# facebookresearch/metamorph

Measured on AMD Instinct MI355X. Metric: train tokens/sec (LLaMA-3-8B + SigLIP-SO400M, seq2048, 256 img toks), whole job, higher is better.
Workload: dtype bf16

## Files before the change

### metamorph_amd/build.py

```python
from __future__ import annotations

import hashlib
import os
import subprocess
import sys

PKG = os.path.dirname(os.path.abspath(__file__))
CSRC = os.path.join(PKG, "csrc")
LIBDIR = os.path.join(PKG, "lib")
LIB = os.path.join(LIBDIR, "libmm355.so")
SOURCES = ["gemm_bf16.hip", "rowwise.hip", "elementwise.hip", "attn.hip", "attn2.hip", "attn4.hip", "attn4_bwd.hip", "decode.hip", "attn_decode.hip", "decode_w8.hip", "decode_w4.hip", "decode_kv8.hip", "attn_extend.hip", "attn_extend_shared.hip", "gemm_w8.hip", "gemm_w4.hip", "greedy.hip", "sample.hip", "logits.hip", "beam.hip", "losses.hip", "linear_ce.hip"]
HEADERS = ["mm355_common.h", "gemm_common.h", "splitk.h", "gemm_wq.h", "decode_wq.h", "attn2.h", "attn_tile.h", "rowsum.h", "argrows.h"] + sorted(
    os.path.join(d, f) for d in ("attn4_gen", "attn4_bwd_gen")
    for f in os.listdir(os.path.join(CSRC, d)) if f.endswith(".inc"))
BASE_FLAGS = ["--offload-arch=gfx950", "-O3", "-std=c++17", "-fPIC", "-Wno-unused-result"]
FLAGS = BASE_FLAGS + ["-mllvm", "-amdgpu-mfma-vgpr-form=1"]
FLAGS_OF = {f: BASE_FLAGS + ["-mllvm", "-amdgpu-spill-vgpr-to-agpr=0"] for f in ("attn4.hip", "attn4_bwd.hip")}


def _hipcc():
    for c in (os.environ.get("HIPCC"), "/opt/rocm/bin/hipcc", "hipcc"):
        if c and (os.path.isabs(c) and os.path.exists(c) or not os.path.isabs(c)):
            return c
    raise RuntimeError("hipcc not found")


def _digest():
    h = hashlib.sha256()
    for f in SOURCES + HEADERS:
        h.update(open(os.path.join(CSRC, f), "rb").read())
    h.update(open(os.path.join(os.path.dirname(PKG), "include", "mm355.h"), "rb").read())
    h.update(" ".join(FLAGS).encode())
    h.update(repr(sorted(FLAGS_OF.items())).encode())
    return h.hexdigest()


def build(force: bool = False, verbose: bool = True) -> str:
    os.makedirs(LIBDIR, exist_ok=True)
    stamp = os.path.join(LIBDIR, "libmm355.stamp")
    dig = _digest()
    if not force and os.path.exists(LIB) and os.path.exists(stamp) and open(stamp).read().strip() == dig:
        return LIB
    hipcc = _hipcc()
    objs = []
    procs = []
    for src in SOURCES:
        obj = os.path.join(LIBDIR, src.replace(".hip", ".o"))
        cmd = [hipcc, *FLAGS_OF.get(src, FLAGS), "-c", os.path.join(CSRC, src), "-o", obj]
        if verbose:
            print("[mm355 build]", " ".join(cmd), flush=True)
        procs.append((src, subprocess.Popen(cmd, stdout=subprocess.PIPE, stderr=subprocess.STDOUT)))
        objs.append(obj)
    for src, p in procs:
        out, _ = p.communicate()
        if p.returncode != 0:
            raise RuntimeError(f"hipcc failed on {src}:\n{out.decode(errors='replace')}")
    cmd = [hipcc, "--offload-arch=gfx950", "-shared", "-fPIC", "-o", LIB, *objs]
    if verbose:
        print("[mm355 build]", " ".join(cmd), flush=True)
    subprocess.check_call(cmd)
    with open(stamp, "w") as f:
        f.write(dig)
    return LIB


if __name__ == "__main__":
    print(build(force="--force" in sys.argv))
```

### metamorph_amd/csrc/gemm_bf16.hip

```cpp
#include "gemm_common.h"
#include "splitk.h"
#include <type_traits>
#include <cstdlib>

namespace {

MM_DEV void gemm_epilogue_swiglu(f32x4 (&acc)[8][4], const GemmArgs& a, unsigned char* smem, int m0, int tn, int wm, int wn, int wave, int lane) {
    constexpr int TN = 64;
    const int fr = lane & 15, fq = lane >> 4;
    const int M = a.M, I = (int)a.res_mod;
    float* stg = (float*)smem + wave * (16 * TN);
    const int row_l = lane >> 2, k4 = lane & 3;
    uint16_t* gu = (uint16_t*)a.C;
    uint16_t* act = (uint16_t*)a.res;
    const int ch0 = tn * 128 + wn * 32;
#pragma unroll
    for (int i = 0; i < 8; ++i) {
        __builtin_amdgcn_fence(__ATOMIC_RELEASE, "wavefront");
        __builtin_amdgcn_wave_barrier();
#pragma unroll
        for (int j = 0; j < 4; ++j)
#pragma unroll
            for (int r = 0; r < 4; ++r) stg[(fq * 4 + r) * TN + j * 16 + fr] = acc[i][j][r];
        __builtin_amdgcn_fence(__ATOMIC_RELEASE, "wavefront");
        __builtin_amdgcn_wave_barrier();
        const int grow = m0 + wm * 128 + i * 16 + row_l;
        if (grow < M) {
            float g[8], u[8], o[8];
            const f32x4 g0 = *(const f32x4*)(stg + row_l * TN + k4 * 8), g1 = *(const f32x4*)(stg + row_l * TN + k4 * 8 + 4);
            const f32x4 u0 = *(const f32x4*)(stg + row_l * TN + 32 + k4 * 8), u1 = *(const f32x4*)(stg + row_l * TN + 32 + k4 * 8 + 4);
            g[0] = g0.x; g[1] = g0.y; g[2] = g0.z; g[3] = g0.w; g[4] = g1.x; g[5] = g1.y; g[6] = g1.z; g[7] = g1.w;
            u[0] = u0.x; u[1] = u0.y; u[2] = u0.z; u[3] = u0.w; u[4] = u1.x; u[5] = u1.y; u[6] = u1.z; u[7] = u1.w;
            const u32x4 gp = pack8(g), up = pack8(u);
            const int ch = ch0 + k4 * 8;
            *(u32x4*)(gu + (int64_t)grow * a.ldc + ch) = gp;
            *(u32x4*)(gu + (int64_t)grow * a.ldc + I + ch) = up;
            float gb[8], ub[8];
            unpack8(gp, gb);
            unpack8(up, ub);
#pragma unroll
            for (int e = 0; e < 8; ++e) o[e] = round_bf(gb[e] / (1.0f + __expf(-gb[e]))) * ub[e];
            *(u32x4*)(act + (int64_t)grow * a.ldr + ch) = pack8(o);
        }
    }
}

constexpr int SWB_TROW = 144;
constexpr int SWB_T = 3 * 32 * SWB_TROW;
constexpr int SWB_LDS = 32768 + 8 * SWB_T;
MM_DEV void gemm_epilogue_swiglu_bwd(f32x4 (&acc)[8][4], const GemmArgs& a, unsigned char* smem, int m0, int n0, int wm, int wn, int wave, int lane) {
    constexpr int TN = 64, PF = 4;
    typedef __attribute__((ext_vector_type(4))) short s16x4;
    typedef __attribute__((address_space(3))) s16x4* lds4_t;
    const int fr = lane & 15, fq = lane >> 4;
    const int M = a.M, I = a.N;
    float* stg = (float*)smem + wave * (16 * TN);
    unsigned char* tile = smem + 32768 + wave * SWB_T;
    const int row_l = lane >> 2, k4 = lane & 3;
    const uint16_t* gu = a.res;
    uint16_t* dgu = (uint16_t*)a.C;
    const int c_wave = n0 + wn * 64;
    if (c_wave >= I) return;
    const int row0 = m0 + wm * 128 + row_l;
    u32x4 gq[PF][2], uq[PF][2];
    auto fetch = [&](int i, int slot) {
        const int grow = row0 + i * 16;
#pragma unroll
        for (int j8 = 0; j8 < 2; ++j8) {
            const int64_t ro = (int64_t)min(grow, M - 1) * a.ldr + c_wave + k4 * 16 + j8 * 8;
            gq[slot][j8] = *(const u32x4*)(gu + ro);
            uq[slot][j8] = *(const u32x4*)(gu + ro + I);
        }
    };
#pragma unroll
    for (int i = 0; i < PF; ++i) fetch(i, i);
#pragma unroll
    for (int ib = 0; ib < 4; ++ib) {
#pragma unroll
        for (int half = 0; half < 2; ++half) {
            const int i = ib * 2 + half;
            __builtin_amdgcn_fence(__ATOMIC_RELEASE, "wavefront");
            __builtin_amdgcn_wave_barrier();
#pragma unroll
            for (int j = 0; j < 4; ++j)
// ... 580 lines not shown
template <int ABL = 0>
__global__ __launch_bounds__(512) void gemm_pp_kernel(GemmArgs a) {
    extern __shared__ __attribute__((aligned(16))) unsigned char smem[];
#ifdef MM355_PP_PERSIST
    const int total = a.ntm * a.ntn;
    for (int bid = blockIdx.x; bid < total; bid += gridDim.x) {
        gemm_pp_tile<ABL>(a, bid, smem);
        __syncthreads();
    }
#else
    gemm_pp_tile<ABL>(a, blockIdx.x, smem);
#endif
}

__global__ __launch_bounds__(512) void gemm_pp_pair_kernel(GemmArgs a0, GemmArgs a1, int n0) {
    extern __shared__ __attribute__((aligned(16))) unsigned char smem[];
    const int bid = blockIdx.x;
    if (bid < n0) gemm_pp_tile(a0, bid, smem);
    else gemm_pp_tile(a1, bid - n0, smem);
}

template <int BM, int BN, int WM, int WN, bool GLDS, int PIPE>
int launch_gemm(GemmArgs a, hipStream_t s);

constexpr int PP_LDS = 2 * (256 + 256) * 128;

int64_t pp_prepare(GemmArgs& a) {
    a.ntm = (a.M + 255) / 256;
    a.ntn = (a.N + 255) / 256;
    a.gm = 4;
    return (int64_t)a.ntm * a.ntn;
}

template <int ABL = 0>
int launch_gemm_pp_t(GemmArgs a, hipStream_t s) {
    static std::atomic<uint64_t> lds_ok{0};
    if (mm_ensure_dynamic_lds((const void*)gemm_pp_kernel<ABL>, PP_LDS, lds_ok) != MM355_OK) return MM355_ELAUNCH;
    const int64_t total = pp_prepare(a);
    if (total <= 0 || total > 0x7fffffff) return MM355_EINVAL;
#ifdef MM355_PP_PERSIST
    hipLaunchKernelGGL((gemm_pp_kernel<ABL>), dim3((unsigned)std::min<int64_t>(total, MM355_PP_PERSIST)), dim3(512), PP_LDS, s, a);
#else
    hipLaunchKernelGGL((gemm_pp_kernel<ABL>), dim3((unsigned)total), dim3(512), PP_LDS, s, a);
#endif
    return mm_launch_status();
}

int launch_gemm_pp_pair(GemmArgs a0, GemmArgs a1, hipStream_t s) {
    static std::atomic<uint64_t> lds_ok{0};
    if (mm_ensure_dynamic_lds((const void*)gemm_pp_pair_kernel, PP_LDS, lds_ok) != MM355_OK) return MM355_ELAUNCH;
    const int64_t n0 = pp_prepare(a0), n1 = pp_prepare(a1);
    if (n0 <= 0 || n1 <= 0 || n0 + n1 > 0x7fffffff) return MM355_EINVAL;
    hipLaunchKernelGGL(gemm_pp_pair_kernel, dim3((unsigned)(n0 + n1)), dim3(512), PP_LDS, s, a0, a1, (int)n0);
    return mm_launch_status();
}

bool pp_eligible(const GemmArgs& a) {
    if (a.K < 128 || (a.K & 127)) return false;
    const int64_t ea = (256 * a.lda + a.K) * 2;
    const int64_t eb = (256 * a.ldb + a.K) * 2;
    return ea < 0x7fffffffLL && eb < 0x7fffffffLL;
}

int launch_gemm_pp(GemmArgs a, hipStream_t s) {
    if (!pp_eligible(a)) return launch_gemm<256, 256, 2, 4, true, 1>(a, s);
    return launch_gemm_pp_t(a, s);
}

template <int BM, int BN, int WM, int WN, bool GLDS, int PIPE = 0>
int launch_gemm(GemmArgs a, hipStream_t s) {
    constexpr int STAGE = (BM + BN) * 128;
    constexpr int LDS = 2 * STAGE;
    auto kern = gemm_nt_kernel<BM, BN, WM, WN, GLDS, PIPE>;
    static std::atomic<uint64_t> lds_ok{0};
    if (mm_ensure_dynamic_lds((const void*)kern, LDS, lds_ok) != MM355_OK) return MM355_ELAUNCH;
    a.ntm = (a.M + BM - 1) / BM;
    a.ntn = (a.N + BN - 1) / BN;
    const int64_t total = (int64_t)a.ntm * a.ntn;
    if (total <= 0 || total > 0x7fffffff) return MM355_EINVAL;
    hipLaunchKernelGGL(kern, dim3((unsigned)total), dim3(WM * WN * 64), LDS, s, a);
    return mm_launch_status();
}

__global__ __launch_bounds__(256) void transpose_kernel(const uint16_t* __restrict__ in, int64_t ld_in, int rows, int cols,
                                                        uint16_t* __restrict__ out, int64_t ld_out) {
    __shared__ uint16_t tile[64][64 + 2];
    const int r0 = blockIdx.y * 64, c0 = blockIdx.x * 64;
    const int tid = threadIdx.x;
#pragma unroll
    for (int i = 0; i < 2; ++i) {
        const int v = tid + i * 256, r = v >> 3, c = (v & 7) * 8;
        const int gr = r0 + r, gc = c0 + c;
        uint16_t tmp[8];
        if (gr < rows && gc + 8 <= cols) {
            *(u32x4*)tmp = *(const u32x4*)(in + (int64_t)gr * ld_in + gc);
        } else {
#pragma unroll
            for (int e = 0; e < 8; ++e) tmp[e] = (gr < rows && gc + e < cols) ? in[(int64_t)gr * ld_in + gc + e] : (uint16_t)0;
        }
#pragma unroll
        for (int e = 0; e < 8; ++e) tile[r][c + e] = tmp[e];
    }
    __syncthreads();
#pragma unroll
    for (int i = 0; i < 2; ++i) {
        const int v = tid + i * 256, c = v >> 3, r = (v & 7) * 8;
        const int gc = c0 + c, gr = r0 + r;
        if (gc >= cols) continue;
        uint16_t tmp[8];
#pragma unroll
        for (int e = 0; e < 8; ++e) tmp[e] = tile[r + e][c];
        if (gr + 8 <= rows && ((ld_out & 7) == 0)) {
            *(u32x4*)(out + (int64_t)gc * ld_out + gr) = *(const u32x4*)tmp;
        } else {
            for (int e = 0; e < 8; ++e)
                if (gr + e < rows) out[(int64_t)gc * ld_out + gr + e] = tmp[e];
        }
    }
}

__global__ __launch_bounds__(256) void colsum_kernel(const uint16_t* __restrict__ x, int64_t ld, int M, int N, float* __restrict__ out) {
    __shared__ float part[4][64];
    const int cq = threadIdx.x & 63, rp = threadIdx.x >> 6;
    const int c = blockIdx.x * 64 + cq;
    float s = 0.f;
    if (c < N)
        for (int r = rp; r < M; r += 4) s += bf2f(x[(int64_t)r * ld + c]);
    part[rp][cq] = s;
    __syncthreads();
    if (rp == 0 && c < N) out[c] += (part[0][cq] + part[1][cq]) + (part[2][cq] + part[3][cq]);
}

__global__ __launch_bounds__(1024) void colsum8_kernel(const uint16_t* __restrict__ x, int64_t ld, int M, int N, float* __restrict__ out) {
    __shared__ float part[128][65];
    const int cg = threadIdx.x & 7, rp = threadIdx.x >> 3;
    const int c0 = blockIdx.x * 64 + cg * 8;
    float s[8] = {0.f, 0.f, 0.f, 0.f, 0.f, 0.f, 0.f, 0.f};
    if (c0 < N)
        for (int r = rp; r < M; r += 128) {
            float f[8];
            unpack8(*(const u32x4*)(x + (int64_t)r * ld + c0), f);
#pragma unroll
            for (int e = 0; e < 8; ++e) s[e] += f[e];
        }
#pragma unroll
    for (int e = 0; e < 8; ++e) part[rp][cg * 8 + e] = s[e];
    __syncthreads();
    const int c = blockIdx.x * 64 + threadIdx.x;
    if (threadIdx.x < 64 && c < N) {
        float t = 0.f;
        for (int p = 0; p < 128; ++p) t += part[p][threadIdx.x];
        out[c] += t;
    }
}

}

namespace {
__global__ __launch_bounds__(256) void splitk_reduce_kernel(const float* __restrict__ part, int S, int M, int N, const uint16_t* __restrict__ res,
                                                            int64_t ldr, uint16_t* __restrict__ out, int64_t ldc) {
    const int nv = N >> 3;
    const int64_t total = (int64_t)M * nv, plane = (int64_t)M * N;
    for (int64_t i = blockIdx.x * 256ll + threadIdx.x; i < total; i += (int64_t)gridDim.x * 256) {
        const int m = (int)(i / nv), c = (int)(i % nv) * 8;
        float v[8];
        const float* p = part + (int64_t)m * N + c;
        const f32x4 a0 = *(const f32x4*)p, a1 = *(const f32x4*)(p + 4);
        v[0] = a0.x; v[1] = a0.y; v[2] = a0.z; v[3] = a0.w; v[4] = a1.x; v[5] = a1.y; v[6] = a1.z; v[7] = a1.w;
        for (int s = 1; s < S; ++s) {
            const f32x4 b0 = *(const f32x4*)(p + s * plane), b1 = *(const f32x4*)(p + s * plane + 4);
            v[0] += b0.x; v[1] += b0.y; v[2] += b0.z; v[3] += b0.w; v[4] += b1.x; v[5] += b1.y; v[6] += b1.z; v[7] += b1.w;
        }
        if (res) {
            float r[8];
            unpack8(*(const u32x4*)(res + (int64_t)m * ldr + c), r);
#pragma unroll
            for (int e = 0; e < 8; ++e) v[e] += r[e];
        }
        *(u32x4*)(out + (int64_t)m * ldc + c) = pack8(v);
    }
}

MM_DEV void splitk_sum8(const float* __restrict__ p, int S, int64_t plane, float (&v)[8]) {
    const f32x4 a0 = *(const f32x4*)p, a1 = *(const f32x4*)(p + 4);
    v[0] = a0.x; v[1] = a0.y; v[2] = a0.z; v[3] = a0.w; v[4] = a1.x; v[5] = a1.y; v[6] = a1.z; v[7] = a1.w;
    int s = 1;
    for (; s + 3 < S; s += 4) {
        f32x4 b0[4], b1[4];
#pragma unroll
        for (int j = 0; j < 4; ++j) { b0[j] = *(const f32x4*)(p + (s + j) * plane); b1[j] = *(const f32x4*)(p + (s + j) * plane + 4); }
#pragma unroll
        for (int j = 0; j < 4; ++j) {
            v[0] += b0[j].x; v[1] += b0[j].y; v[2] += b0[j].z; v[3] += b0[j].w; v[4] += b1[j].x; v[5] += b1[j].y; v[6] += b1[j].z; v[7] += b1[j].w;
        }
    }
    for (; s < S; ++s) {
        const f32x4 b0 = *(const f32x4*)(p + s * plane), b1 = *(const f32x4*)(p + s * plane + 4);
        v[0] += b0.x; v[1] += b0.y; v[2] += b0.z; v[3] += b0.w; v[4] += b1.x; v[5] += b1.y; v[6] += b1.z; v[7] += b1.w;
    }
}
template <int VPT>
// ... 277 lines not shown
        return rc != MM355_OK ? rc : mm355_rope_kv_append(qkv, ld_qkv, M, Hq, Hkv, d, cos_t, sin_t, positions, k_cache, v_cache, ld_kv, batch_stride_kv, stream);
    }
    int slices = 0;
    const int rc = splitk_partials(X, ldx, Wqkv, ldw, M, N, K, S, workspace, workspace_floats, (hipStream_t)stream, slices);
    if (rc != MM355_OK) return rc;
    return mm_splitk_reduce_rope_append(workspace, slices, M, Hq, Hkv, d, qkv, ld_qkv, cos_t, sin_t, positions, k_cache, v_cache, ld_kv,
                                        batch_stride_kv, (hipStream_t)stream);
}

extern "C" int mm355_gemm_num_variants(void) { return 14; }

extern "C" int mm355_gemm_bf16(const mm355_bf16* A, int64_t lda, const mm355_bf16* B, int64_t ldb, void* C, int64_t ldc,
                               int64_t M, int64_t N, int64_t K, const mm355_bf16* bias, const mm355_bf16* residual,
                               int64_t ldr, int64_t res_row_mod, uint32_t flags, int variant, void* stream) {
    (void)hipGetLastError();
    if (!A || !B || !C || M <= 0 || N <= 0 || K <= 0) return MM355_EINVAL;
    if ((K & 7) || (lda & 7) || (ldb & 7) || !mm_aligned16(A) || !mm_aligned16(B) || !mm_aligned16(C)) return MM355_EINVAL;
    if (M > 0x7fffffff || N > 0x7fffffff || K > 0x7fffffff) return MM355_EINVAL;
    if ((flags & MM355_GEMM_BIAS) && (!bias || !mm_aligned16(bias))) return MM355_EINVAL;
    if ((flags & MM355_GEMM_RESIDUAL) && (!residual || !mm_aligned16(residual))) return MM355_EINVAL;
    if ((flags & MM355_GEMM_GELU_ERF) && (flags & MM355_GEMM_GELU_TANH)) return MM355_EINVAL;
    GemmArgs a = {};
    a.A = A; a.B = B; a.C = C; a.bias = bias; a.res = residual;
    a.lda = lda; a.ldb = ldb; a.ldc = ldc; a.ldr = ldr; a.res_mod = res_row_mod;
    a.M = (int)M; a.N = (int)N; a.K = (int)K; a.flags = flags; a.ntm = a.ntn = 0;
    hipStream_t s = (hipStream_t)stream;
    const bool dma_ok = (K % 64) == 0;
    if (variant == 0) {
        const int64_t t256 = ((M + 255) / 256) * ((N + 255) / 256);
        const int64_t t128 = ((M + 127) / 128) * ((N + 127) / 128);
        if (dma_ok) {
            variant = (t256 >= 200) ? 11 : 2;
            if (variant == 2 && t128 < 224 && M > 64 && t128 * 2 >= 64) variant = 9;
        } else variant = 1;
    }
    if (!dma_ok && variant != 1) return MM355_EUNSUPPORTED;
    switch (variant) {
        case 1: return launch_gemm<128, 128, 2, 2, false>(a, s);
        case 2: return launch_gemm<128, 128, 2, 2, true>(a, s);
        case 7: return launch_gemm<256, 256, 2, 4, true, 1>(a, s);
        case 9: return launch_gemm<64, 128, 1, 4, true>(a, s);
        case 11: return launch_gemm_pp(a, s);
#ifdef MM355_ABLATIONS
        case 91: return launch_gemm_pp_t<1>(a, s);
        case 92: return launch_gemm_pp_t<2>(a, s);
        case 93: return launch_gemm_pp_t<3>(a, s);
#endif
        default: return MM355_EUNSUPPORTED;
    }
}

namespace {
int pair_problem(GemmArgs& a, const mm355_bf16* A, int64_t lda, const mm355_bf16* B, int64_t ldb, void* C, int64_t ldc,
                 int64_t M, int64_t N, int64_t K, uint32_t flags) {
    if (!A || !B || !C || M <= 0 || N <= 0 || K <= 0) return MM355_EINVAL;
    if ((K & 7) || (lda & 7) || (ldb & 7) || !mm_aligned16(A) || !mm_aligned16(B) || !mm_aligned16(C)) return MM355_EINVAL;
    if (M > 0x7fffffff || N > 0x7fffffff || K > 0x7fffffff) return MM355_EINVAL;
    if (flags & ~(MM355_GEMM_ACCUMULATE | MM355_GEMM_OUT_F32)) return MM355_EINVAL;
    a.A = A; a.B = B; a.C = C; a.bias = nullptr; a.res = nullptr;
    a.lda = lda; a.ldb = ldb; a.ldc = ldc; a.ldr = 0; a.res_mod = 0;
    a.M = (int)M; a.N = (int)N; a.K = (int)K; a.flags = flags; a.ntm = a.ntn = 0;
    return pp_eligible(a) ? MM355_OK : MM355_EUNSUPPORTED;
}
}

extern "C" int mm355_gemm_pair_bf16(const mm355_bf16* A0, int64_t lda0, const mm355_bf16* B0, int64_t ldb0, void* C0, int64_t ldc0,
                                    int64_t M0, int64_t N0, int64_t K0, uint32_t flags0,
                                    const mm355_bf16* A1, int64_t lda1, const mm355_bf16* B1, int64_t ldb1, void* C1, int64_t ldc1,
                                    int64_t M1, int64_t N1, int64_t K1, uint32_t flags1, void* stream) {
    (void)hipGetLastError();
    GemmArgs a0, a1;
    int rc = pair_problem(a0, A0, lda0, B0, ldb0, C0, ldc0, M0, N0, K0, flags0);
    if (rc != MM355_OK) return rc;
    rc = pair_problem(a1, A1, lda1, B1, ldb1, C1, ldc1, M1, N1, K1, flags1);
    if (rc != MM355_OK) return rc;
    return launch_gemm_pp_pair(a0, a1, (hipStream_t)stream);
}

extern "C" int mm355_transpose_bf16(const mm355_bf16* in, int64_t ld_in, int64_t rows, int64_t cols, mm355_bf16* out,
                                    int64_t ld_out, void* stream) {
    (void)hipGetLastError();
    if (!in || !out || rows <= 0 || cols <= 0 || (ld_in & 7) || !mm_aligned16(in) || !mm_aligned16(out)) return MM355_EINVAL;
    if (ld_out < rows || rows > 0x7fffffff || cols > 0x7fffffff) return MM355_EINVAL;
    dim3 grid((unsigned)((cols + 63) / 64), (unsigned)((rows + 63) / 64));
    hipLaunchKernelGGL(transpose_kernel, grid, dim3(256), 0, (hipStream_t)stream, in, ld_in, (int)rows, (int)cols, out, ld_out);
    return mm_launch_status();
}

extern "C" int mm355_gemm_swiglu_bf16(const mm355_bf16* X, int64_t ldx, const mm355_bf16* Wgu, int64_t ldw, mm355_bf16* gu, int64_t ld_gu,
                                      mm355_bf16* act, int64_t ld_act, int64_t M, int64_t I, int64_t K, void* stream) {
    (void)hipGetLastError();
    if (!X || !Wgu || !gu || !act || M <= 0 || I <= 0 || K <= 0) return MM355_EINVAL;
    if ((ldx & 7) || (ldw & 7) || (ld_gu & 7) || (ld_act & 7) || !mm_aligned16(X) || !mm_aligned16(Wgu) || !mm_aligned16(gu) || !mm_aligned16(act))
        return MM355_EINVAL;
    if (M > 0x7fffffff || I > 0x3fffffff || K > 0x7fffffff) return MM355_EINVAL;
    if ((I & 127) || K < 128 || (K & 127) || (2 * I * ldw + K) * 2 >= 0x7fffffffLL || (256 * ldx + K) * 2 >= 0x7fffffffLL) return MM355_EUNSUPPORTED;
    GemmArgs a = {};
    a.A = X; a.B = Wgu; a.C = gu; a.bias = nullptr; a.res = act;
    a.lda = ldx; a.ldb = ldw; a.ldc = ld_gu; a.ldr = ld_act; a.res_mod = I;
    a.M = (int)M; a.N = (int)(2 * I); a.K = (int)K; a.flags = 0; a.ntm = a.ntn = 0;
    static std::atomic<uint64_t> lds_ok{0};
    if (mm_ensure_dynamic_lds((const void*)gemm_pp_swiglu_kernel, PP_LDS, lds_ok) != MM355_OK) return MM355_ELAUNCH;
    const int64_t total = pp_prepare(a);
    if (total <= 0 || total > 0x7fffffff) return MM355_EINVAL;
    hipLaunchKernelGGL(gemm_pp_swiglu_kernel, dim3((unsigned)total), dim3(512), PP_LDS, (hipStream_t)stream, a);
    return mm_launch_status();
}

extern "C" int mm355_gemm_rope_bf16(const mm355_bf16* X, int64_t ldx, const mm355_bf16* Wqkv, int64_t ldw, mm355_bf16* qkv, int64_t ld_qkv,
                                    const mm355_bf16* cos_t, const mm355_bf16* sin_t, const int32_t* pos_offset,
                                    int64_t M, int64_t N, int64_t K, int64_t L, int64_t n_rot, void* stream) {
    (void)hipGetLastError();
    if (!X || !Wqkv || !qkv || !cos_t || !sin_t || M <= 0 || N <= 0 || K <= 0 || L <= 0 || n_rot < 0 || n_rot > N) return MM355_EINVAL;
    if ((ldx & 7) || (ldw & 7) || (ld_qkv & 7) || !mm_aligned16(X) || !mm_aligned16(Wqkv) || !mm_aligned16(qkv) || !mm_aligned16(cos_t) || !mm_aligned16(sin_t))
        return MM355_EINVAL;
    if (M > 0x7fffffff || N > 0x7fffffff || K > 0x7fffffff || L > 0x7fffffff) return MM355_EINVAL;
    if ((N & 255) || (n_rot & 127) || K < 128 || (K & 127) || (256 * ldx + K) * 2 >= 0x7fffffffLL || (256 * ldw + K) * 2 >= 0x7fffffffLL) return MM355_EUNSUPPORTED;
    GemmArgs a = {};
    a.A = X; a.B = Wqkv; a.C = qkv; a.bias = (const uint16_t*)pos_offset; a.res = nullptr;
    a.lda = ldx; a.ldb = ldw; a.ldc = ld_qkv; a.ldr = 0; a.res_mod = n_rot;
    a.M = (int)M; a.N = (int)N; a.K = (int)K; a.flags = 0; a.ntm = a.ntn = 0;
    a.aux0 = (uint16_t*)cos_t; a.aux1 = (uint16_t*)sin_t; a.ld_aux = L;
    static std::atomic<uint64_t> lds_ok{0};
    if (mm_ensure_dynamic_lds((const void*)gemm_pp_rope_kernel, PP_LDS, lds_ok) != MM355_OK) return MM355_ELAUNCH;
    const int64_t total = pp_prepare(a);
    if (total <= 0 || total > 0x7fffffff) return MM355_EINVAL;
    hipLaunchKernelGGL(gemm_pp_rope_kernel, dim3((unsigned)total), dim3(512), PP_LDS, (hipStream_t)stream, a);
    return mm_launch_status();
}

extern "C" int mm355_gemm_swiglu_bwd_bf16(const mm355_bf16* dY, int64_t ldy, const mm355_bf16* WdT, int64_t ldw, const mm355_bf16* gu, int64_t ld_gu,
                                          mm355_bf16* dgu, int64_t ld_dgu, mm355_bf16* actT, mm355_bf16* dguT, int64_t ldT,
                                          int64_t M, int64_t I, int64_t K, void* stream) {
    (void)hipGetLastError();
    if (!dY || !WdT || !gu || !dgu || !actT || !dguT || M <= 0 || I <= 0 || K <= 0) return MM355_EINVAL;
    if ((ldy & 7) || (ldw & 7) || (ld_gu & 7) || (ld_dgu & 7) || (ldT & 7) || ldT < M || !mm_aligned16(dY) || !mm_aligned16(WdT) || !mm_aligned16(gu)
        || !mm_aligned16(dgu) || !mm_aligned16(actT) || !mm_aligned16(dguT))
        return MM355_EINVAL;
    if (M > 0x7fffffff || I > 0x3fffffff || K > 0x7fffffff) return MM355_EINVAL;
    if ((I & 63) || (M & 7) || K < 128 || (K & 127) || (256 * ldy + K) * 2 >= 0x7fffffffLL || (256 * ldw + K) * 2 >= 0x7fffffffLL) return MM355_EUNSUPPORTED;
    GemmArgs a = {};
    a.A = dY; a.B = WdT; a.C = dgu; a.bias = nullptr; a.res = gu;
    a.lda = ldy; a.ldb = ldw; a.ldc = ld_dgu; a.ldr = ld_gu; a.res_mod = 0;
    a.M = (int)M; a.N = (int)I; a.K = (int)K; a.flags = 0; a.ntm = a.ntn = 0;
    a.aux0 = actT; a.aux1 = dguT; a.ld_aux = ldT;
    static std::atomic<uint64_t> lds_ok{0};
    if (mm_ensure_dynamic_lds((const void*)gemm_pp_swiglu_bwd_kernel, SWB_LDS, lds_ok) != MM355_OK) return MM355_ELAUNCH;
    const int64_t total = pp_prepare(a);
    if (total <= 0 || total > 0x7fffffff) return MM355_EINVAL;
    hipLaunchKernelGGL(gemm_pp_swiglu_bwd_kernel, dim3((unsigned)total), dim3(512), SWB_LDS, (hipStream_t)stream, a);
    return mm_launch_status();
}

extern "C" int mm355_colsum_bf16(const mm355_bf16* dY, int64_t ld, int64_t M, int64_t N, float* db_f32, void* stream) {
    (void)hipGetLastError();
    if (!dY || !db_f32 || M <= 0 || N <= 0) return MM355_EINVAL;
    if (M > 0x7fffffff || N > 0x7fffffff) return MM355_EINVAL;
    if (!(N & 7) && !(ld & 7) && mm_aligned16(dY) && M >= 256)
        hipLaunchKernelGGL(colsum8_kernel, dim3((unsigned)((N + 63) / 64)), dim3(1024), 0, (hipStream_t)stream, dY, ld, (int)M, (int)N, db_f32);
    else
        hipLaunchKernelGGL(colsum_kernel, dim3((unsigned)((N + 63) / 64)), dim3(256), 0, (hipStream_t)stream, dY, ld, (int)M, (int)N, db_f32);
    return mm_launch_status();
}
```

### metamorph_amd/csrc/rowwise.hip

```cpp
#include "mm355_common.h"
#include "rowsum.h"
#include <type_traits>

namespace {

constexpr int NT = 256;

template <int VPT>
__global__ __launch_bounds__(NT) void rmsnorm_fwd_kernel(const uint16_t* __restrict__ x, const uint16_t* __restrict__ w,
                                                         uint16_t* __restrict__ y, float* __restrict__ rstd_out, int h, float eps) {
    __shared__ float red[NT / 64];
    const int64_t row = blockIdx.x;
    const int nv = h >> 3;
    const uint16_t* xr = x + row * h;
    float xv[VPT][8];
    float ss = 0.f;
#pragma unroll
    for (int i = 0; i < VPT; ++i) {
        const int v = threadIdx.x + i * NT;
        if (v < nv) {
            unpack8(*(const u32x4*)(xr + v * 8), xv[i]);
#pragma unroll
            for (int e = 0; e < 8; ++e) ss += xv[i][e] * xv[i][e];
        }
    }
    ss = block_sum<NT>(ss, red);
    const float rstd = rsqrtf(ss / (float)h + eps);
    if (rstd_out && threadIdx.x == 0) rstd_out[row] = rstd;
#pragma unroll
    for (int i = 0; i < VPT; ++i) {
        const int v = threadIdx.x + i * NT;
        if (v < nv) {
            float wv[8], o[8];
            unpack8(*(const u32x4*)(w + v * 8), wv);
#pragma unroll
            for (int e = 0; e < 8; ++e) o[e] = wv[e] * round_bf(xv[i][e] * rstd);
            *(u32x4*)(y + row * h + v * 8) = pack8(o);
        }
    }
}

__global__ __launch_bounds__(256) void rmsnorm_apply_t_kernel(const uint16_t* __restrict__ x, const uint16_t* __restrict__ w,
                                                              const float* __restrict__ rstd, int M, int h,
                                                              uint16_t* __restrict__ out, int64_t ld_out) {
    __shared__ uint16_t tile[64][64 + 2];
    const int r0 = blockIdx.y * 64, c0 = blockIdx.x * 64;
    const int tid = threadIdx.x;
#pragma unroll
    for (int i = 0; i < 2; ++i) {
        const int v = tid + i * 256, r = v >> 3, c = (v & 7) * 8;
        const int gr = r0 + r, gc = c0 + c;
        uint16_t tmp[8];
        if (gr < M && gc + 8 <= h) {
            float xv[8], wv[8], o[8];
            unpack8(*(const u32x4*)(x + (int64_t)gr * h + gc), xv);
            unpack8(*(const u32x4*)(w + gc), wv);
            const float rs = rstd[gr];
#pragma unroll
            for (int e = 0; e < 8; ++e) o[e] = wv[e] * round_bf(xv[e] * rs);
            *(u32x4*)tmp = pack8(o);
        } else {
#pragma unroll
            for (int e = 0; e < 8; ++e) tmp[e] = 0;
        }
#pragma unroll
        for (int e = 0; e < 8; ++e) tile[r][c + e] = tmp[e];
    }
    __syncthreads();
#pragma unroll
    for (int i = 0; i < 2; ++i) {
        const int v = tid + i * 256, c = v >> 3, r = (v & 7) * 8;
        const int gc = c0 + c, gr = r0 + r;
        if (gc >= h) continue;
        uint16_t tmp[8];
#pragma unroll
        for (int e = 0; e < 8; ++e) tmp[e] = tile[r + e][c];
        if (gr + 8 <= M && ((ld_out & 7) == 0)) {
            *(u32x4*)(out + (int64_t)gc * ld_out + gr) = *(const u32x4*)tmp;
        } else {
            for (int e = 0; e < 8; ++e)
                if (gr + e < M) out[(int64_t)gc * ld_out + gr + e] = tmp[e];
        }
    }
}

template <int VPT>
__global__ __launch_bounds__(NT) void rmsnorm_bwd_kernel(const uint16_t* __restrict__ dy, const uint16_t* __restrict__ x,
                                                         const uint16_t* __restrict__ w, const uint16_t* __restrict__ dres,
                                                         uint16_t* __restrict__ dx, float* __restrict__ dw,
                                                         float* __restrict__ ws, int M, int h, float eps, int rows_per_block) {
    __shared__ float red[NT / 64];
    const int nv = h >> 3;
    float wv[VPT][8], dwacc[VPT][8];
#pragma unroll
    for (int i = 0; i < VPT; ++i) {
        const int v = threadIdx.x + i * NT;
#pragma unroll
        for (int e = 0; e < 8; ++e) { dwacc[i][e] = 0.f; wv[i][e] = 0.f; }
        if (v < nv) unpack8(*(const u32x4*)(w + v * 8), wv[i]);
    }
    const int r0 = blockIdx.x * rows_per_block, r1 = min(M, r0 + rows_per_block);
    for (int row = r0; row < r1; ++row) {
        const uint16_t* xr = x + (int64_t)row * h;
        const uint16_t* gr = dy + (int64_t)row * h;
        float xv[VPT][8], gv[VPT][8];
        float ss = 0.f;
#pragma unroll
        for (int i = 0; i < VPT; ++i) {
            const int v = threadIdx.x + i * NT;
            if (v < nv) {
                unpack8(*(const u32x4*)(xr + v * 8), xv[i]);
                unpack8(*(const u32x4*)(gr + v * 8), gv[i]);
#pragma unroll
                for (int e = 0; e < 8; ++e) ss += xv[i][e] * xv[i][e];
            }
        }
        ss = block_sum<NT>(ss, red);
        const float rstd = rsqrtf(ss / (float)h + eps);
        float dot = 0.f;
#pragma unroll
        for (int i = 0; i < VPT; ++i) {
            const int v = threadIdx.x + i * NT;
            if (v < nv) {
#pragma unroll
                for (int e = 0; e < 8; ++e) {
                    const float xh = xv[i][e] * rstd;
                    dwacc[i][e] += gv[i][e] * round_bf(xh);
                    gv[i][e] *= wv[i][e];
                    dot += gv[i][e] * xh;
                }
            }
        }
        dot = block_sum<NT>(dot, red) / (float)h;
#pragma unroll
        for (int i = 0; i < VPT; ++i) {
            const int v = threadIdx.x + i * NT;
            if (v < nv) {
                float o[8];
                if (dres) unpack8(*(const u32x4*)(dres + (int64_t)row * h + v * 8), o);
                else {
#pragma unroll
                    for (int e = 0; e < 8; ++e) o[e] = 0.f;
                }
#pragma unroll
                for (int e = 0; e < 8; ++e) o[e] += rstd * (gv[i][e] - xv[i][e] * rstd * dot);
                *(u32x4*)(dx + (int64_t)row * h + v * 8) = pack8(o);
            }
        }
    }
    if (ws) {
        float* wr = ws + (int64_t)blockIdx.x * h;
#pragma unroll
        for (int i = 0; i < VPT; ++i) {
            const int v = threadIdx.x + i * NT;
            if (v < nv) {
                *(f32x4*)(wr + v * 8) = f32x4{dwacc[i][0], dwacc[i][1], dwacc[i][2], dwacc[i][3]};
                *(f32x4*)(wr + v * 8 + 4) = f32x4{dwacc[i][4], dwacc[i][5], dwacc[i][6], dwacc[i][7]};
            }
        }
    } else if (dw) {
#pragma unroll
        for (int i = 0; i < VPT; ++i) {
            const int v = threadIdx.x + i * NT;
            if (v < nv) {
#pragma unroll
                for (int e = 0; e < 8; ++e) atomicAdd(dw + v * 8 + e, dwacc[i][e]);
// ... 314 lines not shown
    else { lerp_src(oy, si, so, y0, y1, ly); lerp_src(ox, si, so, x0, x1, lx); }
    const int64_t base = (int64_t)n * si * si * C;
    const int64_t o00 = base + (int64_t)(y0 * si + x0) * C, o01 = base + (int64_t)(y0 * si + x1) * C;
    const int64_t o10 = base + (int64_t)(y1 * si + x0) * C, o11 = base + (int64_t)(y1 * si + x1) * C;
    const uint16_t* g = dy + (int64_t)tok * C;
    auto interp = [&](int v, float* r) {
        float a[8], bq[8], c[8], d[8];
        unpack8(*(const u32x4*)(in + o00 + v * 8), a);
        unpack8(*(const u32x4*)(in + o01 + v * 8), bq);
        unpack8(*(const u32x4*)(in + o10 + v * 8), c);
        unpack8(*(const u32x4*)(in + o11 + v * 8), d);
#pragma unroll
        for (int e = 0; e < 8; ++e) {
            const float top = a[e] * (1.0f - lx) + bq[e] * lx;
            const float bot = c[e] * (1.0f - lx) + d[e] * lx;
            r[e] = round_bf(si == so ? a[e] : top * (1.0f - ly) + bot * ly);
        }
    };
    float inv = 1.0f, dot = 0.f;
    if (normalize) {
        float ss = 0.f;
        for (int v = lane; v < nv; v += 64) {
            float r[8], gy[8];
            interp(v, r);
            unpack8(*(const u32x4*)(g + v * 8), gy);
#pragma unroll
            for (int e = 0; e < 8; ++e) { ss += r[e] * r[e]; dot += r[e] * gy[e]; }
        }
        ss = wave_sum(ss);
        dot = wave_sum(dot);
        const float nrm = fmaxf(round_bf(sqrtf(ss)), 1e-12f);
        inv = 1.0f / nrm;
        dot *= inv * inv;
    }
    const float w00 = (1.0f - lx) * (1.0f - ly), w01 = lx * (1.0f - ly), w10 = (1.0f - lx) * ly, w11 = lx * ly;
    for (int v = lane; v < nv; v += 64) {
        float r[8], gy[8];
        unpack8(*(const u32x4*)(g + v * 8), gy);
        if (normalize) interp(v, r);
#pragma unroll
        for (int e = 0; e < 8; ++e) {
            const float dr = normalize ? (gy[e] - r[e] * dot) * inv : gy[e];
            if (si == so) atomicAdd(din + o00 + v * 8 + e, dr);
            else {
                atomicAdd(din + o00 + v * 8 + e, dr * w00);
                atomicAdd(din + o01 + v * 8 + e, dr * w01);
                atomicAdd(din + o10 + v * 8 + e, dr * w10);
                atomicAdd(din + o11 + v * 8 + e, dr * w11);
            }
        }
    }
}

template <typename F>
int dispatch_vpt(int h, F&& f) {
    const int nv = h >> 3;
    if (nv <= NT) return f(std::integral_constant<int, 1>{});
    if (nv <= 2 * NT) return f(std::integral_constant<int, 2>{});
    if (nv <= 4 * NT) return f(std::integral_constant<int, 4>{});
    if (nv <= 8 * NT) return f(std::integral_constant<int, 8>{});
    return MM355_EUNSUPPORTED;
}

}

extern "C" int mm355_rmsnorm_fwd_rstd(const mm355_bf16* x, const mm355_bf16* w, mm355_bf16* y, float* rstd_out, int64_t M, int64_t h, float eps,
                                      void* stream) {
    (void)hipGetLastError();
    if (!x || !w || !y || M <= 0 || h <= 0 || (h & 7) || M > 0x7fffffff) return MM355_EINVAL;
    return dispatch_vpt((int)h, [&](auto vpt) {
        hipLaunchKernelGGL((rmsnorm_fwd_kernel<decltype(vpt)::value>), dim3((unsigned)M), dim3(NT), 0, (hipStream_t)stream, x, w, y, rstd_out,
                           (int)h, eps);
        return mm_launch_status();
    });
}
extern "C" int mm355_rmsnorm_fwd(const mm355_bf16* x, const mm355_bf16* w, mm355_bf16* y, int64_t M, int64_t h, float eps, void* stream) {
    return mm355_rmsnorm_fwd_rstd(x, w, y, nullptr, M, h, eps, stream);
}
extern "C" int mm355_rmsnorm_apply_t(const mm355_bf16* x, const mm355_bf16* w, const float* rstd, int64_t M, int64_t h, mm355_bf16* out_t,
                                     int64_t ld_out, void* stream) {
    (void)hipGetLastError();
    if (!x || !w || !rstd || !out_t || M <= 0 || h <= 0 || (h & 7) || M > 0x7fffffff || ld_out < M) return MM355_EINVAL;
    if (!mm_aligned16(x) || !mm_aligned16(w) || !mm_aligned16(out_t)) return MM355_EINVAL;
    dim3 grid((unsigned)((h + 63) / 64), (unsigned)((M + 63) / 64));
    hipLaunchKernelGGL(rmsnorm_apply_t_kernel, grid, dim3(256), 0, (hipStream_t)stream, x, w, rstd, (int)M, (int)h, out_t, ld_out);
    return mm_launch_status();
}

constexpr int DWR_COLS = 32;
__global__ __launch_bounds__(256) void rmsnorm_dw_reduce_kernel(const float* __restrict__ ws, float* __restrict__ dw, int G, int h, int ld) {
    __shared__ f32x4 part[32][8];
    const int cq = threadIdx.x & 7, rl = threadIdx.x >> 3;
    const int c = blockIdx.x * DWR_COLS + cq * 4;
    f32x4 acc0 = {0.f, 0.f, 0.f, 0.f}, acc1 = {0.f, 0.f, 0.f, 0.f};
    if (c < h) {
        const float* p = ws + c;
        int g = rl;
        for (; g + 32 < G; g += 64) {
            acc0 += *(const f32x4*)(p + (int64_t)g * ld);
            acc1 += *(const f32x4*)(p + (int64_t)(g + 32) * ld);
        }
        if (g < G) acc0 += *(const f32x4*)(p + (int64_t)g * ld);
    }
    part[rl][cq] = acc0 + acc1;
    __syncthreads();
    if (rl == 0 && c < h) {
        f32x4 s = part[0][cq];
#pragma unroll
        for (int r = 1; r < 32; ++r) s += part[r][cq];
#pragma unroll
        for (int e = 0; e < 4; ++e) dw[c + e] += s[e];
    }
}

__global__ __launch_bounds__(256) void rmsnorm_dw_reduce_bf16_kernel(const float* __restrict__ ws, uint16_t* __restrict__ grad, int G, int h, int ld,
                                                                     int accumulate) {
    __shared__ f32x4 part[32][8];
    const int cq = threadIdx.x & 7, rl = threadIdx.x >> 3;
    const int c = blockIdx.x * DWR_COLS + cq * 4;
    f32x4 acc0 = {0.f, 0.f, 0.f, 0.f}, acc1 = {0.f, 0.f, 0.f, 0.f};
    if (c < h) {
        const float* p = ws + c;
        int g = rl;
        for (; g + 32 < G; g += 64) {
            acc0 += *(const f32x4*)(p + (int64_t)g * ld);
            acc1 += *(const f32x4*)(p + (int64_t)(g + 32) * ld);
        }
        if (g < G) acc0 += *(const f32x4*)(p + (int64_t)g * ld);
    }
    part[rl][cq] = acc0 + acc1;
    __syncthreads();
    if (rl == 0 && c < h) {
        f32x4 s = part[0][cq];
#pragma unroll
        for (int r = 1; r < 32; ++r) s += part[r][cq];
#pragma unroll
        for (int e = 0; e < 4; ++e) grad[c + e] = f2bf(s[e] + (accumulate ? bf2f(grad[c + e]) : 0.f));
    }
}

static int rmsnorm_bwd_rows_per_block(int64_t M, bool two_stage) {
    if (two_stage) return M >= 8192 ? 32 : (M >= 1024 ? 8 : 1);
    return M >= 8192 ? 16 : (M >= 1024 ? 4 : 1);
}

extern "C" int64_t mm355_rmsnorm_bwd_ws_floats(int64_t M, int64_t h) {
    if (M <= 0 || h <= 0) return 0;
    const int rpb = rmsnorm_bwd_rows_per_block(M, true);
    return ((M + rpb - 1) / rpb) * h;
}

extern "C" int mm355_rmsnorm_bwd(const mm355_bf16* dy, const mm355_bf16* x, const mm355_bf16* w, const mm355_bf16* dres,
                                 mm355_bf16* dx, float* dw_f32, float* workspace, int64_t M, int64_t h, float eps, void* stream) {
    (void)hipGetLastError();
    if (!dy || !x || !w || !dx || M <= 0 || h <= 0 || (h & 7) || M > 0x7fffffff) return MM355_EINVAL;
    const bool two_stage = dw_f32 && workspace;
    if (two_stage && !mm_aligned16(workspace)) return MM355_EINVAL;
    const int rpb = rmsnorm_bwd_rows_per_block(M, two_stage);
    const unsigned grid = (unsigned)((M + rpb - 1) / rpb);
    int rc = dispatch_vpt((int)h, [&](auto vpt) {
        hipLaunchKernelGGL((rmsnorm_bwd_kernel<decltype(vpt)::value>), dim3(grid), dim3(NT), 0, (hipStream_t)stream, dy, x, w, dres, dx,
                           dw_f32, two_stage ? workspace : nullptr, (int)M, (int)h, eps, rpb);
        return mm_launch_status();
    });
    if (rc != MM355_OK || !two_stage) return rc;
    hipLaunchKernelGGL(rmsnorm_dw_reduce_kernel, dim3((unsigned)((h + DWR_COLS - 1) / DWR_COLS)), dim3(256), 0, (hipStream_t)stream, workspace, dw_f32,
                       (int)grid, (int)h, (int)h);
    return mm_launch_status();
// ... 104 lines not shown
```

Measured before the change: 26550.

## Share transpose tile helper using swizzled LDS and ds_read_tr16 transposed reads

Replaces the hand-written 64x64 padded-LDS transposes in the generic transpose and rmsnorm_apply_t kernels with a shared header. The header uses 128x64 tiles, an XOR-swizzled LDS layout, gfx950 ds_read_tr16_b64 transposed LDS reads, and a diagonal 1D block-to-tile mapping meant to spread traffic across memory channels. It aims to cut LDS bank conflicts and per-element scalar LDS accesses, and to vectorize the stores. The cost is a more intricate lane mapping that must be correct at tile edges.

```diff
diff --git a/metamorph_amd/build.py b/metamorph_amd/build.py
--- a/metamorph_amd/build.py
+++ b/metamorph_amd/build.py
@@ -10,7 +10,7 @@
 LIBDIR = os.path.join(PKG, "lib")
 LIB = os.path.join(LIBDIR, "libmm355.so")
 SOURCES = ["gemm_bf16.hip", "rowwise.hip", "elementwise.hip", "attn.hip", "attn2.hip", "attn4.hip", "attn4_bwd.hip", "decode.hip", "attn_decode.hip", "decode_w8.hip", "decode_w4.hip", "decode_kv8.hip", "attn_extend.hip", "attn_extend_shared.hip", "gemm_w8.hip", "gemm_w4.hip", "greedy.hip", "sample.hip", "logits.hip", "beam.hip", "losses.hip", "linear_ce.hip"]
-HEADERS = ["mm355_common.h", "gemm_common.h", "splitk.h", "gemm_wq.h", "decode_wq.h", "attn2.h", "attn_tile.h", "rowsum.h", "argrows.h"] + sorted(
+HEADERS = ["mm355_common.h", "gemm_common.h", "splitk.h", "gemm_wq.h", "decode_wq.h", "attn2.h", "attn_tile.h", "rowsum.h", "argrows.h", "transpose_tile.h"] + sorted(
     os.path.join(d, f) for d in ("attn4_gen", "attn4_bwd_gen")
     for f in os.listdir(os.path.join(CSRC, d)) if f.endswith(".inc"))
 BASE_FLAGS = ["--offload-arch=gfx950", "-O3", "-std=c++17", "-fPIC", "-Wno-unused-result"]
diff --git a/metamorph_amd/csrc/gemm_bf16.hip b/metamorph_amd/csrc/gemm_bf16.hip
--- a/metamorph_amd/csrc/gemm_bf16.hip
+++ b/metamorph_amd/csrc/gemm_bf16.hip
@@ -1,5 +1,6 @@
 #include "gemm_common.h"
 #include "splitk.h"
+#include "transpose_tile.h"
 #include <type_traits>
 #include <cstdlib>
 
@@ -746,41 +747,20 @@
     return mm_launch_status();
 }
 
+constexpr int TT_ROWS = MM355_TT_ROWS, TT_COLS = MM355_TT_COLS;
 __global__ __launch_bounds__(256) void transpose_kernel(const uint16_t* __restrict__ in, int64_t ld_in, int rows, int cols,
                                                         uint16_t* __restrict__ out, int64_t ld_out) {
-    __shared__ uint16_t tile[64][64 + 2];
-    const int r0 = blockIdx.y * 64, c0 = blockIdx.x * 64;
-    const int tid = threadIdx.x;
-#pragma unroll
-    for (int i = 0; i < 2; ++i) {
-        const int v = tid + i * 256, r = v >> 3, c = (v & 7) * 8;
-        const int gr = r0 + r, gc = c0 + c;
+    __shared__ __attribute__((aligned(16))) unsigned char lds[tt::Tile<TT_ROWS, TT_COLS>::BYTES];
+    int tr, tc;
+    tt::tile_of_block((rows + TT_ROWS - 1) / TT_ROWS, (cols + TT_COLS - 1) / TT_COLS, tr, tc);
+    tt::transpose_tile<TT_ROWS, TT_COLS>(lds, tr * TT_ROWS, tc * TT_COLS, rows, cols, out, ld_out,
+                                         [&](int gr, int gc, bool interior) -> u32x4 {
+        if (interior || (gr < rows && gc + 8 <= cols)) return *(const u32x4*)(in + (int64_t)gr * ld_in + gc);
         uint16_t tmp[8];
-        if (gr < rows && gc + 8 <= cols) {
-            *(u32x4*)tmp = *(const u32x4*)(in + (int64_t)gr * ld_in + gc);
-        } else {
-#pragma unroll
-            for (int e = 0; e < 8; ++e) tmp[e] = (gr < rows && gc + e < cols) ? in[(int64_t)gr * ld_in + gc + e] : (uint16_t)0;
-        }
-#pragma unroll
-        for (int e = 0; e < 8; ++e) tile[r][c + e] = tmp[e];
-    }
-    __syncthreads();
-#pragma unroll
-    for (int i = 0; i < 2; ++i) {
-        const int v = tid + i * 256, c = v >> 3, r = (v & 7) * 8;
-        const int gc = c0 + c, gr = r0 + r;
-        if (gc >= cols) continue;
-        uint16_t tmp[8];
-#pragma unroll
-        for (int e = 0; e < 8; ++e) tmp[e] = tile[r + e][c];
-        if (gr + 8 <= rows && ((ld_out & 7) == 0)) {
-            *(u32x4*)(out + (int64_t)gc * ld_out + gr) = *(const u32x4*)tmp;
-        } else {
-            for (int e = 0; e < 8; ++e)
-                if (gr + e < rows) out[(int64_t)gc * ld_out + gr + e] = tmp[e];
-        }
-    }
+#pragma unroll
+        for (int e = 0; e < 8; ++e) tmp[e] = (gr < rows && gc + e < cols) ? in[(int64_t)gr * ld_in + gc + e] : (uint16_t)0;
+        return *(const u32x4*)tmp;
+    });
 }
 
 __global__ __launch_bounds__(256) void colsum_kernel(const uint16_t* __restrict__ x, int64_t ld, int M, int N, float* __restrict__ out) {
@@ -1224,8 +1204,9 @@
     (void)hipGetLastError();
     if (!in || !out || rows <= 0 || cols <= 0 || (ld_in & 7) || !mm_aligned16(in) || !mm_aligned16(out)) return MM355_EINVAL;
     if (ld_out < rows || rows > 0x7fffffff || cols > 0x7fffffff) return MM355_EINVAL;
-    dim3 grid((unsigned)((cols + 63) / 64), (unsigned)((rows + 63) / 64));
-    hipLaunchKernelGGL(transpose_kernel, grid, dim3(256), 0, (hipStream_t)stream, in, ld_in, (int)rows, (int)cols, out, ld_out);
+    const int64_t tiles = ((cols + TT_COLS - 1) / TT_COLS) * ((rows + TT_ROWS - 1) / TT_ROWS);
+    if (tiles > 0x7fffffff) return MM355_EINVAL;
+    hipLaunchKernelGGL(transpose_kernel, dim3((unsigned)tiles), dim3(256), 0, (hipStream_t)stream, in, ld_in, (int)rows, (int)cols, out, ld_out);
     return mm_launch_status();
 }
 
diff --git a/metamorph_amd/csrc/rowwise.hip b/metamorph_amd/csrc/rowwise.hip
--- a/metamorph_amd/csrc/rowwise.hip
+++ b/metamorph_amd/csrc/rowwise.hip
@@ -1,5 +1,6 @@
 #include "mm355_common.h"
 #include "rowsum.h"
+#include "transpose_tile.h"
 #include <type_traits>
 
 namespace {
@@ -40,48 +41,24 @@
     }
 }
 
+constexpr int TT_ROWS = MM355_TT_ROWS, TT_COLS = MM355_TT_COLS;
 __global__ __launch_bounds__(256) void rmsnorm_apply_t_kernel(const uint16_t* __restrict__ x, const uint16_t* __restrict__ w,
                                                               const float* __restrict__ rstd, int M, int h,
                                                               uint16_t* __restrict__ out, int64_t ld_out) {
-    __shared__ uint16_t tile[64][64 + 2];
-    const int r0 = blockIdx.y * 64, c0 = blockIdx.x * 64;
-    const int tid = threadIdx.x;
-#pragma unroll
-    for (int i = 0; i < 2; ++i) {
-        const int v = tid + i * 256, r = v >> 3, c = (v & 7) * 8;
-        const int gr = r0 + r, gc = c0 + c;
-        uint16_t tmp[8];
-        if (gr < M && gc + 8 <= h) {
-            float xv[8], wv[8], o[8];
-            unpack8(*(const u32x4*)(x + (int64_t)gr * h + gc), xv);
-            unpack8(*(const u32x4*)(w + gc), wv);
-            const float rs = rstd[gr];
-#pragma unroll
-            for (int e = 0; e < 8; ++e) o[e] = wv[e] * round_bf(xv[e] * rs);
-            *(u32x4*)tmp = pack8(o);
-        } else {
-#pragma unroll
-            for (int e = 0; e < 8; ++e) tmp[e] = 0;
-        }
-#pragma unroll
-        for (int e = 0; e < 8; ++e) tile[r][c + e] = tmp[e];
-    }
-    __syncthreads();
-#pragma unroll
-    for (int i = 0; i < 2; ++i) {
-        const int v = tid + i * 256, c = v >> 3, r = (v & 7) * 8;
-        const int gc = c0 + c, gr = r0 + r;
-        if (gc >= h) continue;
-        uint16_t tmp[8];
-#pragma unroll
-        for (int e = 0; e < 8; ++e) tmp[e] = tile[r + e][c];
-        if (gr + 8 <= M && ((ld_out & 7) == 0)) {
-            *(u32x4*)(out + (int64_t)gc * ld_out + gr) = *(const u32x4*)tmp;
-        } else {
-            for (int e = 0; e < 8; ++e)
-                if (gr + e < M) out[(int64_t)gc * ld_out + gr + e] = tmp[e];
-        }
-    }
+    __shared__ __attribute__((aligned(16))) unsigned char lds[tt::Tile<TT_ROWS, TT_COLS>::BYTES];
+    int tr, tc;
+    tt::tile_of_block((M + TT_ROWS - 1) / TT_ROWS, (h + TT_COLS - 1) / TT_COLS, tr, tc);
+    tt::transpose_tile<TT_ROWS, TT_COLS>(lds, tr * TT_ROWS, tc * TT_COLS, M, h, out, ld_out,
+                                         [&](int gr, int gc, bool interior) -> u32x4 {
+        if (!interior && (gr >= M || gc >= h)) return u32x4{0u, 0u, 0u, 0u};
+        float xv[8], wv[8], o[8];
+        unpack8(*(const u32x4*)(x + (int64_t)gr * h + gc), xv);
+        unpack8(*(const u32x4*)(w + gc), wv);
+        const float rs = rstd[gr];
+#pragma unroll
+        for (int e = 0; e < 8; ++e) o[e] = wv[e] * round_bf(xv[e] * rs);
+        return pack8(o);
+    });
 }
 
 template <int VPT>
@@ -562,8 +539,9 @@
     (void)hipGetLastError();
     if (!x || !w || !rstd || !out_t || M <= 0 || h <= 0 || (h & 7) || M > 0x7fffffff || ld_out < M) return MM355_EINVAL;
     if (!mm_aligned16(x) || !mm_aligned16(w) || !mm_aligned16(out_t)) return MM355_EINVAL;
-    dim3 grid((unsigned)((h + 63) / 64), (unsigned)((M + 63) / 64));
-    hipLaunchKernelGGL(rmsnorm_apply_t_kernel, grid, dim3(256), 0, (hipStream_t)stream, x, w, rstd, (int)M, (int)h, out_t, ld_out);
+    const int64_t tiles = ((h + TT_COLS - 1) / TT_COLS) * ((M + TT_ROWS - 1) / TT_ROWS);
+    if (tiles > 0x7fffffff) return MM355_EINVAL;
+    hipLaunchKernelGGL(rmsnorm_apply_t_kernel, dim3((unsigned)tiles), dim3(256), 0, (hipStream_t)stream, x, w, rstd, (int)M, (int)h, out_t, ld_out);
     return mm_launch_status();
 }
 
diff --git a/metamorph_amd/csrc/transpose_tile.h b/metamorph_amd/csrc/transpose_tile.h
--- /dev/null
+++ b/metamorph_amd/csrc/transpose_tile.h
@@ -0,0 +1,112 @@
+#pragma once
+#include "mm355_common.h"
+
+namespace tt {
+
+typedef __attribute__((ext_vector_type(4))) short s16x4;
+typedef __attribute__((ext_vector_type(8))) short s16x8;
+typedef __attribute__((address_space(3))) s16x4* lds4_t;
+
+#ifndef MM355_TT_ROWS
+#define MM355_TT_ROWS 128
+#endif
+#ifndef MM355_TT_COLS
+#define MM355_TT_COLS 64
+#endif
+
+#ifndef MM355_TT_ORDER
+#define MM355_TT_ORDER (-1)
+#endif
+MM_DEV void tile_of_block(int ntr, int ntc, int& tr, int& tc) {
+    const int id = blockIdx.x;
+    if (MM355_TT_ORDER < 0) {
+        if (MM355_TT_ORDER == -1) {
+            const int d = id / ntr;
+            tr = id - d * ntr, tc = (d + tr) % ntc;
+        } else {
+            const int d = id / ntc;
+            tc = id - d * ntc, tr = (d + tc) % ntr;
+        }
+    } else if (MM355_TT_ORDER == 0) {
+        tr = id / ntc, tc = id - tr * ntc;
+    } else if (MM355_TT_ORDER == 1) {
+        tc = id / ntr, tr = id - tc * ntr;
+    } else {
+        const int per = MM355_TT_ORDER * ntc, grp = id / per, in = id - grp * per;
+        const int g = min(MM355_TT_ORDER, ntr - grp * MM355_TT_ORDER);
+        tc = in / g, tr = grp * MM355_TT_ORDER + (in - tc * g);
+    }
+}
+
+template <int TR, int TC>
+struct Tile {
+    static_assert((TR == 64 || TR == 128) && (TC == 64 || TC == 128), "tile shapes the unit walk below covers");
+    static constexpr int NT = 256;
+    static constexpr int CPR = TC / 8;
+    static constexpr int PITCH = TC * 2;
+    static constexpr int BYTES = TR * PITCH;
+    static constexpr int NLOAD = TR * CPR / NT;
+    static constexpr int RB = TR / 64;
+    static constexpr int UPW = RB * CPR / 4;
+    static MM_DEV int swz(int row) {
+        return TC == 64 ? (((row >> 1) & 1) | (((row >> 3) & 3) << 1)) : ((row & 3) | (((row >> 3) & 3) << 2));
+    }
+    static MM_DEV int off(int row, int ch) { return row * PITCH + ((ch ^ swz(row)) << 4); }
+};
+
+template <int TR, int TC, class Load>
+MM_DEV void transpose_tile(unsigned char* lds, int r0, int c0, int rows, int cols, uint16_t* __restrict__ out, int64_t ld_out, Load load) {
+    using T = Tile<TR, TC>;
+    const int tid = threadIdx.x;
+    const bool interior = r0 + TR <= rows && c0 + TC <= cols;
+    const int ch_w = tid % T::CPR, r_w = tid / T::CPR;
+    u32x4 v[T::NLOAD];
+    if (interior) {
+#pragma unroll
+        for (int i = 0; i < T::NLOAD; ++i) v[i] = load(r0 + r_w + i * (T::NT / T::CPR), c0 + ch_w * 8, true);
+    } else {
+#pragma unroll
+        for (int i = 0; i < T::NLOAD; ++i) v[i] = load(r0 + r_w + i * (T::NT / T::CPR), c0 + ch_w * 8, false);
+    }
+    const int wave = tid >> 6, lane = tid & 63, g = lane >> 4, n = lane & 15;
+    const int srow = 32 * (g >> 1) + 8 * (n & 3) + (n >> 2);
+    const int rrow = 32 * (g >> 1) + 8 * (n >> 2), rcol = 4 * (g & 1) + (n & 3);
+    s16x8 t[T::UPW];
+#ifdef MM355_TT_NOLDS
+    static_assert(T::UPW == T::NLOAD, "one store per load");
+#pragma unroll
+    for (int u = 0; u < T::UPW; ++u) t[u] = __builtin_bit_cast(s16x8, v[u]);
+#else
+#pragma unroll
+    for (int i = 0; i < T::NLOAD; ++i) *(u32x4*)(lds + T::off(r_w + i * (T::NT / T::CPR), ch_w)) = v[i];
+    __syncthreads();
+#pragma unroll
+    for (int u = 0; u < T::UPW; ++u) {
+        const int unit = wave * T::UPW + u, ch = unit / T::RB, rb = (unit % T::RB) * 64;
+        const unsigned char* p = lds + T::off(rb + srow, ch) + 8 * (g & 1);
+        const s16x4 lo = __builtin_amdgcn_ds_read_tr16_b64_v4i16((lds4_t)p);
+        const s16x4 hi = __builtin_amdgcn_ds_read_tr16_b64_v4i16((lds4_t)(p + 4 * T::PITCH));
+        t[u] = s16x8{lo[0], lo[1], lo[2], lo[3], hi[0], hi[1], hi[2], hi[3]};
+    }
+#endif
+    const bool vec_out = (ld_out & 7) == 0;
+#pragma unroll
+    for (int u = 0; u < T::UPW; ++u) {
+        const int unit = wave * T::UPW + u, ch = unit / T::RB, rb = (unit % T::RB) * 64;
+        const int gc = c0 + ch * 8 + rcol, gr = r0 + rb + rrow;
+        uint16_t* o = out + (int64_t)gc * ld_out + gr;
+        if (interior && vec_out) {
+            *(s16x8*)o = t[u];
+        } else if (gc < cols) {
+            if (vec_out && gr + 8 <= rows) {
+                *(s16x8*)o = t[u];
+            } else {
+#pragma unroll
+                for (int e = 0; e < 8; ++e)
+                    if (gr + e < rows) o[e] = (uint16_t)t[u][e];
+            }
+        }
+    }
+}
+
+}
```

After: 26570 (median of 2 runs). Within noise of the previous version (+0.0%).
